# tranqkhue/bugcar_image_segmentation

Hardware: AMD Instinct MI355X
Metric: frames/sec ENet 640x480 segmentation -> BEV occupancy grid (synthetic), whole job (higher is better)
Workload: dtype fp32; 1 GPU; config3/5: ENet 640x480 batch 64 per GPU, preprocess + forward + argmax/LUT + fused BEV warp/occgrid (1000x1000 BEV -> 200x200 cells); global_batch=64, per_gpu_batch=64, height=480, width=640, parallelism=frame-sharded dp1, streams_per_gpu=1, hip_graph=True, ranks=1, devices=1, backend=none (one process)

## Files before the change

__graft_entry__.py:

```python
from __future__ import annotations

import os
import sys

ROOT = os.path.dirname(os.path.abspath(__file__))
if ROOT not in sys.path:
    sys.path.insert(0, ROOT)


def build() -> None:
    from bugcar_image_segmentation_amd.build import build_native
    build_native()
    from oracle.build import build_oracle
    build_oracle()
    import bugcar_image_segmentation_amd
    from bugcar_image_segmentation_amd import _native
    _native.load_library()


def smoke() -> None:
    import numpy as np
    import torch
    from bugcar_image_segmentation_amd import enet_spec, synthetic
    from bugcar_image_segmentation_amd.models import ENET
    from bugcar_image_segmentation_amd.pipeline import OccupancyPipeline
    from oracle import ocv_c

    assert torch.cuda.is_available(), "smoke() needs cuda:0"
    torch.cuda.set_device(0)
    blocks = enet_spec.build_enet()
    H, W = 96, 128
    frames = synthetic.road_frames(2, H, W, seed=3)
    bev = synthetic.synthetic_bev(H, W, 200, 200)
    grid = (4.0, 4.0, 0.05)
    model = ENET(weights=blocks, precision="fp32")
    pipe = OccupancyPipeline(model, bev, *grid, model_hw=(H, W))
    out = pipe.run(torch.from_numpy(frames).cuda()).cpu().numpy()
    x = np.concatenate([ENET.preprocess_device(f, width=W, height=H).cpu().numpy() for f in frames])
    logits = model.logits(x)
    cls_ref, grids_ref, logits_ref = ocv_c.pipeline(frames, blocks, bev._bev_matrix, 200, 200, 1.0, grid, (H, W))
    err = float(np.abs(logits - logits_ref).max())
    assert err < 1e-3, f"logits differ from the oracle by {err}"
    s = np.sort(logits_ref, axis=1)
    thr = max(2.5 * err, 1e-5)
    decided = (s[:, -1] - s[:, -2]) > thr
    cls = model.predict(x)
    assert (cls[decided] == cls_ref[decided]).all(), "class map differs from the oracle"
    seg = pipe._seg.cpu().numpy()
    assert (seg[decided] == cls_ref[decided]).all(), "pipeline class map differs from the oracle"
    own = np.stack([ocv_c.create_occupancy_grid(c, bev._bev_matrix, 200, 200, 1.0, *grid) for c in seg])
    assert (out == own).all(), "occupancy grid differs from the oracle's rasteriser on the same class map"
    from bugcar_image_segmentation_amd import deeplab_spec
    from bugcar_image_segmentation_amd.models import DeepLabV3
    from oracle import deeplab_oracle
    net = deeplab_spec.build_deeplab(width=0.25, crop=65)
    dl = DeepLabV3(net=net, precision="fp32")
    rgb = np.random.default_rng(4).integers(0, 256, (1, 65, 60, 3), dtype=np.uint8)
    seg = dl.predict(rgb)
    dl_logits = dl.logits_device().cpu().numpy()[..., :net.num_classes].transpose(0, 3, 1, 2)
    dl_err = float(np.abs(dl_logits - deeplab_oracle.forward(net, rgb).numpy()).max())
    assert dl_err < 1e-3, f"DeepLab logits differ from the oracle by {dl_err}"
    assert np.array_equal(seg, deeplab_oracle.predict(net, rgb, logits=dl_logits)), "DeepLab resize/argmax differs"
    from bugcar_image_segmentation_amd.models import class_lut3
    net2 = deeplab_spec.build_deeplab(width=0.25, crop=(65, 97))
    dl2 = DeepLabV3(net=net2, precision="fp32")
# ... 91 lines not shown
```

bugcar_image_segmentation_amd/build.py:

```python
from __future__ import annotations

import os
import subprocess
import sys
from concurrent.futures import ThreadPoolExecutor
from pathlib import Path

PKG = Path(__file__).resolve().parent
ROOT = PKG.parent
CSRC = PKG / "csrc"
OBJ = PKG / "_build"
LIB = PKG / "libbugseg.so"
SOURCES = ["conv_kernels.hip", "cls_kernels.hip", "init_kernels.hip", "bneck_kernels.hip", "bneck2_kernels.hip", "up_kernels.hip", "prep_kernels.hip",
           "bev_kernels.hip", "deeplab_kernels.hip", "bugseg_runtime.cpp", "deeplab_runtime.cpp"]
HEADERS = [CSRC / "bugseg_internal.h", CSRC / "deeplab_internal.h", CSRC / "knobs.h", CSRC / "mfma_common.h", CSRC / "cls_common.h", ROOT / "include" / "bugseg.h"]
ARCH = os.environ.get("BUGSEG_OFFLOAD_ARCH", "gfx950")
SOURCE_FLAGS = {"cls_kernels.hip": ["-mllvm", "-amdgpu-mfma-vgpr-form=1"]}


def _hipcc() -> str:
    for c in (os.environ.get("HIPCC"), "/opt/rocm/bin/hipcc", "hipcc"):
        if c and (os.path.sep not in c or os.path.exists(c)):
            return c
    raise RuntimeError("hipcc not found")


def _stale(target: Path, deps) -> bool:
    if not target.exists():
        return True
    t = target.stat().st_mtime
    return any(Path(d).stat().st_mtime > t for d in deps)


def build_native(force: bool = False, verbose: bool = False, stamps: bool = False, variant: str = "",
                 defines=()) -> Path:
    if stamps:
        variant, defines = "stamps", ("-DBUGSEG_STAMPS", *defines)
    obj_dir = OBJ / variant if variant else OBJ
    lib = PKG / f"libbugseg_{variant}.so" if variant else LIB
    obj_dir.mkdir(parents=True, exist_ok=True)
    hipcc = _hipcc()
    flags = [f"--offload-arch={ARCH}", "-O3", "-std=c++17", "-fPIC", "-Wall", "-Wno-unused-function",
             f"-I{ROOT / 'include'}", f"-I{CSRC}", *defines]
    jobs = []
    for s in SOURCES:
        src = CSRC / s
        obj = obj_dir / (s + ".o")
        if force or _stale(obj, [src, *HEADERS]):
            lang = ["-x", "hip"] if s.endswith(".hip") else []
            jobs.append((obj, [hipcc, *flags, *SOURCE_FLAGS.get(s, []), *lang, "-c", str(src), "-o", str(obj)]))

    def run(job):
        obj, cmd = job
        if verbose:
            print(" ".join(cmd), file=sys.stderr)
        r = subprocess.run(cmd, capture_output=True, text=True)
        if r.returncode != 0:
            raise RuntimeError(f"compile failed: {' '.join(cmd)}\n{r.stdout}\n{r.stderr}")
        return obj

    with ThreadPoolExecutor(max_workers=min(4, max(1, len(jobs)))) as ex:
        list(ex.map(run, jobs))
    objs = [obj_dir / (s + ".o") for s in SOURCES]
    if force or jobs or _stale(lib, objs):
        tmp = lib.with_suffix(".so.tmp")
        cmd = [hipcc, f"--offload-arch={ARCH}", "-shared", "-fPIC", "-o", str(tmp), *map(str, objs)]
        r = subprocess.run(cmd, capture_output=True, text=True)
        if r.returncode != 0:
            raise RuntimeError(f"link failed: {' '.join(cmd)}\n{r.stdout}\n{r.stderr}")
        os.replace(tmp, lib)
    return lib


if __name__ == "__main__":
    var = next((a.split("=", 1)[1] for a in sys.argv if a.startswith("--variant=")), "")
    print(build_native(force="--force" in sys.argv, verbose=True, stamps="--stamps" in sys.argv, variant=var,
                       defines=tuple(a for a in sys.argv if a.startswith("-D"))))
```

bugcar_image_segmentation_amd/csrc/bneck_kernels.hip:

```cpp
#include <algorithm>
#include <cstdlib>

#include <type_traits>

#include "bugseg_internal.h"
#ifndef BUGSEG_OUT_AUX
#define BUGSEG_OUT_AUX -1
#endif
#include "cls_common.h"

namespace bugseg {

#ifdef BUGSEG_STAMPS
__device__ unsigned long long *bugseg_stamps;
#define STAMP(k) do { if (tid == 0 && bugseg_stamps) bugseg_stamps[(size_t)tile * 8 + (k)] = __builtin_amdgcn_s_memtime(); } while (0)
#define STAMP_WG() do { if (tid == 0 && bugseg_stamps) bugseg_stamps[(size_t)tile * 8 + 7] = blockIdx.x; } while (0)
#define STAMP_ENTRY(k) do { if (threadIdx.x == 0 && bugseg_stamps) bugseg_stamps[(1u << 19) + 2u * blockIdx.x + (k)] = __builtin_amdgcn_s_memrealtime(); } while (0)
#else
#define STAMP_ENTRY(k) do {} while (0)
#define STAMP(k) do {} while (0)
#define STAMP_WG() do {} while (0)
#endif

__device__ __forceinline__ void vm_wait_upto(int n) {
#define VMW(k) case k: asm volatile("s_waitcnt vmcnt(" #k ")" ::: "memory"); break;
    switch (n) {
        VMW(2) VMW(4) VMW(6) VMW(8) VMW(10) VMW(12) VMW(14) VMW(16) VMW(18) VMW(20) VMW(22) VMW(24)
        default: asm volatile("s_waitcnt vmcnt(0)" ::: "memory"); break;
    }
#undef VMW
}

template <int C, int V> struct BShape;
template <> struct BShape<128, 0> { static constexpr int TH = 16, TW = 16, NW = 8, OCC = 4, RP = 2, RD = 0, WIDE = 1; };
template <> struct BShape<128, 1> { static constexpr int TH = 20, TW = 16, NW = 8, OCC = 4, RP = 2, RD = 0, WIDE = 1; };
template <> struct BShape<128, 2> { static constexpr int TH = 4, TW = 80, NW = 8, OCC = 4, RP = 2, RD = 1, WIDE = 0; };
template <> struct BShape<128, 3> { static constexpr int TH = 4, TW = 64, NW = 8, OCC = 4, RP = 2, RD = 1, WIDE = 1; };
template <> struct BShape<128, 4> { static constexpr int TH = 8, TW = 16, NW = 8, OCC = 4, RP = 1, RD = 0, WIDE = 1; };
template <> struct BShape<64, 0> { static constexpr int TH = 16, TW = 16, NW = 4, OCC = 5, RP = 4, RD = 0, WIDE = 1; };
template <> struct BShape<64, 2> { static constexpr int TH = 8, TW = 16, NW = 4, OCC = 5, RP = 2, RD = 0, WIDE = 1; };
template <> struct BShape<64, 1> { static constexpr int TH = 20, TW = 16, NW = 4, OCC = 5, RP = 3, RD = 0, WIDE = 1; };
template <> struct BShape<16, 0> { static constexpr int TH = 16, TW = 16, NW = 4, OCC = 6, RP = 4, RD = 0, WIDE = 1; };
template <> struct BShape<16, 1> { static constexpr int TH = 20, TW = 16, NW = 4, OCC = 6, RP = 4, RD = 0, WIDE = 1; };

#ifndef BNECK_F32_HL
#define BNECK_F32_HL 1
#endif
#ifndef BNECK_F32_HL64
#define BNECK_F32_HL64 1
#endif
__host__ __device__ constexpr bool bneck_hl(int es, int C, bool dn) {
    return BNECK_F32_HL && es == 4 && (C == 128 || (C == 64 && BNECK_F32_HL64)) && !dn;
}
__host__ __device__ constexpr bool bneck_pl(int es, int C, bool dn) { return bneck_hl(es, C, dn) && C == 64; }
__host__ __device__ constexpr int bneck_padw(int es, int C, bool wide, bool dn) {
    return bneck_hl(es, C, dn) ? 8 : es == 2 && (C != 128 || wide) ? 16 : 16 / es;
}
__host__ __device__ constexpr int bneck_pstr(int es, int IS, bool wide) {
    return es != 2 ? (BNECK_F32_HL && es == 4 && IS == 32 ? 40 : IS + 16 / es) : IS == 32 ? (wide ? 48 : 40) : IS;
}
static bool bneck_wide(int C, int v, bool asym) {
#define BW_CASE(CC, VV) if (C == CC && v == VV) return BShape<CC, VV>::WIDE && !asym;
    BW_CASE(128, 0) BW_CASE(128, 1) BW_CASE(128, 2) BW_CASE(128, 3) BW_CASE(128, 4) BW_CASE(64, 0) BW_CASE(64, 1) BW_CASE(64, 2) BW_CASE(16, 0) BW_CASE(16, 1)
#undef BW_CASE
    return false;
}

int bneck_variants(int C) { return C == 128 ? 6 : C == 16 ? 2 : 3; }

void bneck_shape(int C, int v, int &th, int &tw, int &nw, int *rd) {
    if (C == 128 && v == BNECK2_V) { th = 16; tw = 16; nw = 16; if (rd) *rd = 0; return; }
#define BS_CASE(CC, VV) if (C == CC && v == VV) { th = BShape<CC, VV>::TH; tw = BShape<CC, VV>::TW; nw = BShape<CC, VV>::NW; if (rd) *rd = BShape<CC, VV>::RD; return; }
    BS_CASE(128, 0) BS_CASE(128, 1) BS_CASE(128, 2) BS_CASE(128, 3) BS_CASE(128, 4) BS_CASE(64, 0) BS_CASE(64, 1) BS_CASE(64, 2) BS_CASE(16, 0) BS_CASE(16, 1)
#undef BS_CASE
    th = tw = nw = 0;
    if (rd) *rd = 0;
}

#ifndef BNECK_F32_SPLIT_T0
#define BNECK_F32_SPLIT_T0 1
#endif
#ifndef BNECK_F32_OCC16
#define BNECK_F32_OCC16 4
#endif
// ... 72 lines not shown
#define BNECK_PH2_UNROLL 0
#endif
#ifndef BNECK_ASYM_UNROLL
#define BNECK_ASYM_UNROLL 1
#endif
#ifndef BNECK_REG3_C64
#define BNECK_REG3_C64 0
#endif
#ifndef BNECK_F32_LINES64
#define BNECK_F32_LINES64 0
#endif
#ifndef BNECK_REG3_C64_F32
#define BNECK_REG3_C64_F32 0
#endif
#ifndef BNECK_F32_HSTG
#define BNECK_F32_HSTG 1
#endif
#ifndef BNECK_CH1_C64
#define BNECK_CH1_C64 6
#endif
#ifndef BNECK_CH1_K8
#define BNECK_CH1_K8 1
#endif
#ifndef BNECK_CH1_K8_F32
#define BNECK_CH1_K8_F32 1
#endif
    constexpr int CH1 = KS1 >= 8 ? (sizeof(T) == 4 ? BNECK_CH1_K8_F32 : BNECK_CH1_K8) : KS1 >= 4 ? (NF1 + NW - 1) / NW
                    : KS1 == 2 ? (C == 64 && V == 0 && !DN && !ASYM ? BNECK_CH1_C64 : BNECK_CH1_K2) : 8;
    constexpr bool REG3 = C != 64 || DN || BNECK_REG3_C64 || (sizeof(T) == 4 && (BNECK_REG3_C64_F32 || BNECK_F32_LINES64));
    constexpr bool SWAP = REG3 && sizeof(T) == 2 && NR3 % 2 == 0;
    constexpr bool HALF = REG3 && sizeof(T) == 2 && NR3 % 2 != 0;
    constexpr int EPC = 16 / (int)sizeof(T);
    constexpr int CPP = C / EPC;
    constexpr int CPF = 16 * CPP;
    constexpr int CPL = (CPF + 63) / 64;
    constexpr bool HSTG = !REG3 && sizeof(T) == 4 && C == 64 && BNECK_F32_HSTG;
    constexpr int OSTR = (HSTG ? C / 2 : C) + EPC;
    constexpr int RQ3 = !REG3 ? CPL : SWAP ? NR3 / 2 : NR3;
    static_assert(TW % 16 == 0, "a fragment is a run of one tile row");
#ifndef BNECK_NBE
#define BNECK_NBE -1
#endif
#ifndef BNECK_KEEP
#define BNECK_KEEP 1
#endif
#ifndef BNECK_GLDS
#define BNECK_GLDS 1
#endif
#ifndef BNECK_CONST_GLDS
#define BNECK_CONST_GLDS 1
#endif
#ifndef BNECK_GLDS_PARTIAL
#define BNECK_GLDS_PARTIAL 1
#endif
    constexpr bool GLDS = BNECK_GLDS;
#ifndef BNECK_KEEP_ASYM
#define BNECK_KEEP_ASYM 1
#endif
#ifndef BNECK_KEEP_C64
#define BNECK_KEEP_C64 1
#endif
#ifndef BNECK_KEEP_F32
#define BNECK_KEEP_F32 1
#endif
#ifndef BNECK_KEEP_F32_ASYM
#define BNECK_KEEP_F32_ASYM 1
#endif
    constexpr bool KEEPF = BNECK_KEEP_F32 && !DN && sizeof(T) == 4 && (!ASYM || BNECK_KEEP_F32_ASYM) && C == 128 && REG3 && !SWAP;
    constexpr bool KEEP = (BNECK_KEEP && !DN && sizeof(T) == 2 && (!ASYM || BNECK_KEEP_ASYM) && (SWAP || !REG3) && (C != 64 || BNECK_KEEP_C64) &&
                           NF2 * KS1 * 4 <= (C == 128 ? 48 : 32)) || KEEPF;
    static_assert(!KEEP || !REG3 || (KEEPF ? 2 * KS1 == RQ3 : KS1 == RQ3), "kept x: one 16-B chunk per k-step and row pair");
#ifndef BNECK_EARLY_FREE
#define BNECK_EARLY_FREE 0
#endif
    constexpr bool EARLY_FREE = BNECK_EARLY_FREE && KEEP && REG3;
#ifndef BNECK_DKEEP
#define BNECK_DKEEP 1
#endif
#ifndef BNECK_DKEEP_F32
#define BNECK_DKEEP_F32 1
#endif
    constexpr bool DKEEP = BNECK_DKEEP && DN && ((sizeof(T) == 2 && SWAP) || (sizeof(T) == 4 && BNECK_DKEEP_F32 && REG3));
    constexpr int NPK = DN ? (CI + 31) / 32 : 1;
    constexpr int PKW = sizeof(T) == 4 ? 2 : 1;
#ifndef BNECK_F32_LINES
#define BNECK_F32_LINES 1
#endif
    constexpr bool LINES64 = BNECK_F32_LINES64 && sizeof(T) == 4 && REG3 && C == 64 && !DN && !KEEP;
    constexpr bool LINES = (BNECK_F32_LINES && sizeof(T) == 4 && REG3 && C == 128 && (KEEPF || (DKEEP && PKW == 2)) && RQ3 % 2 == 0) ||
                           LINES64;
    constexpr bool CLS = FC >= 0;
    static_assert(!CLS || (C == 16 && !ASYM && !DN && !TR && REG3 && !KEEP && !SWAP && TH == 16 && TW == 16 && NW == 4),
                  "class fusion: the 16 x 16 C16 form");
    constexpr int OPS = sizeof(T) == 4 ? 20 : 24;
    extern __shared__ __attribute__((aligned(16))) unsigned char smem[];
    using SRaw = typename std::conditional<sizeof(T) == 4 && BNECK_F32_SPLIT_T0, RawS, Raw>::type;
    constexpr bool HL = bneck_hl((int)sizeof(T), C, CI > 0) && !(C == 64 && ASYM);
    static_assert(!HL || (BNECK_F32_SPLIT_T0 && (IS == 32 || (PL && IS == 16)) && BNECK_GLDS), "HL: split t0 of 32 channels (PL: 16), LDS-DMA staging");
    constexpr int PLO = PL ? HR * PSTR : 0;
    constexpr int ZP = HL ? 32 : 16;
    auto st4t = [](T *p, int ch, float4 v) {
        if constexpr (PL) {
            const float e[4] = {v.x, v.y, v.z, v.w};
            _Float16 hh[4], ll[4];
#pragma unroll
            for (int i = 0; i < 4; ++i) {
                hh[i] = (_Float16)e[i];
                ll[i] = (_Float16)(e[i] - (float)hh[i]);
            }
            unsigned char *b = reinterpret_cast<unsigned char *>(reinterpret_cast<float *>(p) - ch) + (ch >> 3) * 16 + (ch & 7) * 2;
            *reinterpret_cast<f16x4 *>(b) = (f16x4){hh[0], hh[1], hh[2], hh[3]};
            *reinterpret_cast<f16x4 *>(b + PLO * 4) = (f16x4){ll[0], ll[1], ll[2], ll[3]};
        } else if constexpr (HL) st4hl(reinterpret_cast<float *>(p) - ch, ch, v);
        else if constexpr (sizeof(T) == 4 && BNECK_F32_SPLIT_T0) st4s(reinterpret_cast<float *>(p) - (ch & 7), ch & 7, v);
        else st4(p, v);
    };

    span_enter(a.span);
    STAMP_ENTRY(0);
    {
        if (tile_walk((int)(blockIdx.x & 7), (int)(blockIdx.x >> 3), tile_walk_ch(a.ntiles), a.ntiles, a.rev) < 0) return true;
    }
    const int tid = threadIdx.x;
    const int lane = tid & 63, col = lane & 15, kq = lane >> 4;
    const int wave = __builtin_amdgcn_readfirstlane(tid >> 6);
    auto chunk_ch = [&](int t) -> int { return SWAP ? (2 * t + (kq & 1)) * 16 + 8 * (kq >> 1) : t * 16 + kq * 4; };
    const int K1S = KS1 * 32 + PADW, K2S = KS2 * 32 + PADW, K3S = 32 + PADW;
    auto ldw = [&](WRaw &r, const T *p) {
        if constexpr (HL) {
            r.h = *reinterpret_cast<const uint4 *>(p + kq * 4);
            r.l = *reinterpret_cast<const uint4 *>(p + 16 + kq * 4);
        } else {
            ld8(r, p + kq * 8);
        }
    };
    T *w1 = reinterpret_cast<T *>(smem);
    T *w2 = w1 + NR1 * 16 * K1S;
    T *w2b = w2 + NR1 * 16 * K2S;
    T *w3 = w2b + (ASYM ? NR1 * 16 * K2S : 0);
    constexpr int NP1 = NR1 * 16;
    float *cb1 = reinterpret_cast<float *>(w3 + C * K3S), *cs1 = cb1 + NP1, *cb2 = cs1 + NP1, *cs2 = cb2 + NP1;
    float *cb2b = cs2 + NP1, *cs2b = cb2b + NP1, *cb3 = cs2b + NP1, *cs3 = cb3 + C, *cso = cs3 + C;
    T *zpad = reinterpret_cast<T *>(cso + C);
    T *ts = zpad + ZP;
    float *wmx = reinterpret_cast<float *>(ts + HR * PSTR);
    T *otile = ts + HR * PSTR;
    uint4 *cwl = reinterpret_cast<uint4 *>(otile + (CLS ? NPX * OPS : 0));
    float *cbl = reinterpret_cast<float *>(cwl + (CLS ? (sizeof(T) == 4 ? 1024 : 512) : 0));
    float *cmx = cbl + 64;
    {
        constexpr int CPR1 = KS1 * 32 * (int)sizeof(T) / 16, CPR2 = KS2 * 32 * (int)sizeof(T) / 16, CPR3 = 32 * (int)sizeof(T) / 16;
        constexpr int N1 = NR1 * 16 * CPR1, N2 = NR1 * 16 * CPR2, N3 = C * CPR3;
        constexpr int TOT = N1 + N2 * (ASYM ? 2 : 1) + N3;
        constexpr int PER = (TOT + NT - 1) / NT;
        uint4 buf[C == 16 ? PER : 1];
        auto locate = [&](int i, const uint4 *&src, unsigned char *&dst) -> bool {
            int r, c;
            if (i < N1) { r = i / CPR1; c = i - r * CPR1; src = (const uint4 *)a.w1 + i; dst = (unsigned char *)(w1 + r * K1S) + c * 16; return true; }
            i -= N1;
            if (i < N2) { r = i / CPR2; c = i - r * CPR2; src = (const uint4 *)a.w2 + i; dst = (unsigned char *)(w2 + r * K2S) + c * 16; return true; }
            i -= N2;
            if (ASYM && i < N2) { r = i / CPR2; c = i - r * CPR2; src = (const uint4 *)a.w2b + i; dst = (unsigned char *)(w2b + r * K2S) + c * 16; return true; }
            if (ASYM) i -= N2;
            if (i < N3) { r = i / CPR3; c = i - r * CPR3; src = (const uint4 *)a.w3 + i; dst = (unsigned char *)(w3 + r * K3S) + c * 16; return true; }
            return false;
        };
        if constexpr (GLDS) {
            (void)buf;
            constexpr int ES = (int)sizeof(T);
            constexpr int SR1 = (KS1 * 32 + PADW) * ES / 16, SR2 = (KS2 * 32 + PADW) * ES / 16, SR3 = (32 + PADW) * ES / 16;
            constexpr int S1 = NR1 * 16 * SR1, S2 = NR1 * 16 * SR2, S3 = C * SR3;
            constexpr int NSL = S1 + S2 * (ASYM ? 2 : 1) + S3;
            static_assert((KS1 * 32 + PADW) * ES % 16 == 0 && (KS2 * 32 + PADW) * ES % 16 == 0 && (32 + PADW) * ES % 16 == 0,
                          "weight rows are whole 16-B slots");
            for (int base = wave * 64; base < NSL; base += NT) {
                const int q = base + lane;
                const uint4 *src;
                auto pick = [&](const void *w, int k, int SR, int CPR) {
                    const int r = k / SR, c = k - r * SR;
                    const int cs = HL ? (c & ~7) | ((c & 7) < 4 ? 2 * (c & 7) : 2 * (c & 3) + 1) : c;
                    src = (const uint4 *)w + r * CPR + (c < CPR ? cs : 0);
                };
                constexpr int O3 = S1 + S2 * (ASYM ? 2 : 1);
                if (q < S1) pick(a.w1, q, SR1, CPR1);
                else if (q < S1 + S2) pick(a.w2, q - S1, SR2, CPR2);
                else if (q < O3) pick(a.w2b, q - S1 - S2, SR2, CPR2);
                else pick(a.w3, q - O3, SR3, CPR3);
                if (base + lane < NSL)
                    __builtin_amdgcn_global_load_lds((__attribute__((address_space(1))) void *)src,
                                                     (__attribute__((address_space(3))) void *)(smem + (size_t)base * 16), 16, 0, 0);
            }
        } else if constexpr (C == 16) {
#pragma unroll
            for (int k = 0; k < PER; ++k) {
                const uint4 *src;
                unsigned char *dst;
                if (locate(tid + k * NT, src, dst)) buf[k] = *src;
            }
#pragma unroll
            for (int k = 0; k < PER; ++k) {
                const uint4 *src;
                unsigned char *dst;
                if (locate(tid + k * NT, src, dst)) *reinterpret_cast<uint4 *>(dst) = buf[k];
            }
        } else {
            (void)buf;
            for (int i = tid; i < TOT; i += NT) {
                const uint4 *src;
                unsigned char *dst;
                if (locate(i, src, dst)) *reinterpret_cast<uint4 *>(dst) = *src;
            }
        }
        if constexpr (GLDS && (BNECK_CONST_GLDS == 2 || (BNECK_CONST_GLDS == 1 && C != 128))) {
            const float *srcs[9] = {a.b1, a.s1, a.b2, a.s2, a.b2b, a.s2b, a.b3, a.s3, a.s_out};
            float *dsts[9] = {cb1, cs1, cb2, cs2, cb2b, cs2b, cb3, cs3, cso};
            int item = 0;
#pragma unroll
            for (int k = 0; k < 9; ++k) {
                if (!ASYM && (k == 4 || k == 5)) continue;
                const int n = k < 6 ? NP1 : C;
#pragma unroll
                for (int c0 = 0; c0 < n; c0 += 64, ++item) {
                    if (item % NW != wave) continue;
                    if (c0 + lane < n)
                        __builtin_amdgcn_global_load_lds((__attribute__((address_space(1))) void *)(srcs[k] + c0 + lane),
                                                         (__attribute__((address_space(3))) void *)(dsts[k] + c0), 4, 0, 0);
                }
            }
        } else {
            for (int i = tid; i < NP1; i += NT) {
                cb1[i] = a.b1[i]; cs1[i] = a.s1[i]; cb2[i] = a.b2[i]; cs2[i] = a.s2[i];
                cb2b[i] = ASYM ? a.b2b[i] : 0.f; cs2b[i] = ASYM ? a.s2b[i] : 0.f;
            }
            for (int i = tid; i < C; i += NT) { cb3[i] = a.b3[i]; cs3[i] = a.s3[i]; cso[i] = a.s_out[i]; }
        }
        if (tid < ZP) zpad[tid] = (T)0.f;
    }
    using CRaw = typename WTr<T>::Raw;
    uint64_t lut64 = 0;
    bool cshort[2] = {false, false};
    if constexpr (CLS) {
        const T *cw = reinterpret_cast<const T *>(a.cw);
        for (int q = tid; q < 512; q += NT) {
            const int bs = q >> 6, ln = q & 63;
            const T *src = cw + (size_t)cls_prow(bs >> 2, ln & 31) * 64 + (bs & 3) * 16 + 8 * (ln >> 5);
            if constexpr (sizeof(T) == 4) {
                cwl[q] = reinterpret_cast<const uint4 *>(src)[0];
                cwl[512 + q] = reinterpret_cast<const uint4 *>(src)[1];
            } else {
                cwl[q] = *reinterpret_cast<const uint4 *>(src);
            }
        }
        if (tid < 64) cbl[tid] = (tid & 15) < a.ncls ? a.cbias[tid] : -INFINITY;
        lut64 = cls_lut64(a.lut);
#pragma unroll
        for (int b = 0; b < 2; ++b) {
            CRaw w2_, w3_;
            const T *r = cw + (size_t)cls_prow(b, lane & 31) * 64 + 8 * (lane >> 5);
            ld8(w2_, r + 32);
            ld8(w3_, r + 48);
            cshort[b] = __ballot(nonzero(w2_) || nonzero(w3_)) == 0;
        }
    }
    const auto rxb = mkbuf(DN ? a.xin : a.x, DN ? a.xin_bytes : a.x_bytes);
    const auto rob = mkbuf(a.out, a.x_bytes);
    const auto rpb = mkbuf(a.pool, a.pool_bytes);
// ... 159 lines not shown
                    __builtin_amdgcn_raw_buffer_store_b64((u32x2_t){lo, hi}, rib, wr ? (int)(pix * a.idxCS + cc * 8) : (int)OOB, 0, 0);
                };
                auto seq = [](float &bv, int &bp, float v, int p) {
                    const bool t = v > bv;
                    bv = t ? v : bv;
                    bp = t ? p : bp;
                };
                if constexpr (CG1 >= 4) {
#pragma unroll
                    for (int hgrp = 0; hgrp < CG1 / 4; ++hgrp) {
                        float bv[8], e[8];
                        int bp[8];
#pragma unroll
                        for (int i = 0; i < 8; ++i) { bv[i] = -INFINITY; bp[i] = 4; }
#pragma unroll
                        for (int tap = 0; tap < 4; ++tap) {
                            elems(xs[tap * (CG1 / 4) + hgrp], e);
#pragma unroll
                            for (int i = 0; i < 8; ++i) seq(bv[i], bp[i], e[i], tap);
                        }
                        emit(hgrp * 4 + kq, bv, bp, interior, hgrp, true);
                    }
                } else {
                    float bv[8], e[8];
                    int bp[8];
#pragma unroll
                    for (int i = 0; i < 8; ++i) { bv[i] = -INFINITY; bp[i] = 4; }
                    const int dx = kq >> 1;
#pragma unroll
                    for (int dy = 0; dy < 2; ++dy) {
                        elems(xs[dy], e);
#pragma unroll
                        for (int i = 0; i < 8; ++i) seq(bv[i], bp[i], e[i], dy * 2 + dx);
                    }
                    const bool lo_half = kq < 2;
#pragma unroll
                    for (int i = 0; i < 8; ++i) {
                        uint32_t v0 = __float_as_uint(bv[i]), v1 = v0, p0 = (uint32_t)bp[i], p1 = p0;
                        pl32swap(v0, v1);
                        pl32swap(p0, p1);
                        const float pv = __uint_as_float(lo_half ? v1 : v0);
                        const int pp = (int)(lo_half ? p1 : p0);
                        const bool t = pv > bv[i] || (pv == bv[i] && pp < bp[i]);
                        bv[i] = t ? pv : bv[i];
                        bp[i] = t ? pp : bp[i];
                    }
                    emit(kq & 1, bv, bp, interior && lo_half, 0, lo_half);
                }
            }
        };
        STAMP(0); STAMP_WG();
        const bool first = it == slot;
        if constexpr (!KEEP) {
            if (GLDS && first) asm volatile("s_waitcnt vmcnt(0)" ::: "memory");
            __syncthreads();
            if constexpr (F32 && !SCL) {
                if (first && bneck_range<ASYM>(a.rg, rng_reduce(rlane)).any) {
                    asm volatile("s_waitcnt vmcnt(0) lgkmcnt(0)" ::: "memory");
                    __syncthreads();
                    return false;
                }
            }
        }
        STAMP(1);

        auto int_h = [&](int f) -> int {
            const int p = f * 16 + col, i = p / TW, j = p - i * TW;
            return (i + RY) * HWW + j + RX;
        };
        auto load_hg = [&](int ty0, int tx0, uint32_t txn, int h, bool valid, Raw (&xs)[KS1]) -> bool {
            const int hy = h / HWW, hx = h - hy * HWW;
            const int iy = ty0 + dt * ((tr ? hx : hy) - RY), ix = tx0 + dtx * ((tr ? hy : hx) - RX);
            const bool ok = valid && (unsigned)iy < (unsigned)a.H && (unsigned)ix < (unsigned)a.W;
#pragma unroll
            for (int s = 0; s < KS1; ++s) {
                const int g = s * 4 + kq;
                bld8(xs[s], rxb, ok && g < G1 ? txn + ((__umul24((uint32_t)iy, (uint32_t)a.W) + (uint32_t)ix) * C + g * 8) * (uint32_t)sizeof(T) : OOB);
            }
            return ok;
        };
        constexpr int NBD = HR - NPX, NFB = (NBD + 15) / 16;
        constexpr int NBW = (NFB + NW - 1) / NW;
        constexpr int B0 = NFT % NW;
        const int wb = wave >= B0 ? wave - B0 : wave - B0 + NW;
        auto bord_h = [&](int b) -> int {
            if (b < 2 * RY * HWW) {
                const int r = b / HWW, c = b - r * HWW;
                return (r < RY ? r : TH + r) * HWW + c;
            }
            if constexpr (RX > 0) {
                const int bb = b - 2 * RY * HWW, r = bb / (2 * RX), c = bb - r * (2 * RX);
                return (RY + r) * HWW + (c < RX ? c : TW + c);
            }
            return 0;
        };
        auto proj = [&](int h, bool valid, bool ok, const Raw (&xs)[KS1]) {
            f32x4 acc[NR1];
            proj_mfma(acc, xs);
            if (valid) {
#pragma unroll
                for (int r = 0; r < NR1; ++r) {
                    const int ch = r * 16 + kq * 4;
                    if (ch >= IS) continue;
                    float4 v = act(f4(acc[r]), cs1 + ch);
                    if (!ok) v = make_float4(0.f, 0.f, 0.f, 0.f);
                    st4t(ts + h * PSTR + ch, ch, v);
                }
            }
        };
        uint4 pres[DKEEP ? NF2 : 1][NPK * PKW];
        if constexpr (KEEP) {
            auto load_h = [&](int h, bool valid, Raw (&xs)[KS1]) -> bool { return load_hg(oy0, ox0, xn, h, valid, xs); };
            Raw bx[NBW][KS1];
            int bh[NBW];
            bool bok[NBW];
            if (!pref) {
#pragma unroll
                for (int j = 0; j < NF2; ++j)
                    if (wave + NW * j < NFT && need1(wave + NW * j)) kok[j] = load_h(int_h(wave + NW * j), true, kx[j]);
            }
            auto load_b = [&](int k) {
                const int b = (wb + NW * k) * 16 + col;
                bh[k] = b < NBD ? bord_h(b) : 0;
                bok[k] = load_h(bh[k], b < NBD, bx[k]);
            };
            constexpr int NBE = BNECK_NBE >= 0 ? BNECK_NBE : C == 128 && !RD && !ASYM && sizeof(T) == 2 ? 1 : 0;
#pragma unroll
            for (int k = 0; k < NBE && k < NBW; ++k)
                if (wb + NW * k < NFB && needb(wb + NW * k)) load_b(k);
            if (GLDS && first) {
                int nld = 0;
                constexpr int LPS = sizeof(T) == 4 ? 2 : 1;
#pragma unroll
                for (int j = 0; j < NF2; ++j) nld += wave + NW * j < NFT && need1(wave + NW * j) ? KS1 * LPS : 0;
#pragma unroll
                for (int k = 0; k < NBE && k < NBW; ++k) nld += wb + NW * k < NFB && needb(wb + NW * k) ? KS1 * LPS : 0;
                vm_wait_upto(BNECK_GLDS_PARTIAL ? (nld < 24 ? nld & ~1 : 24) : 0);
            }
            asm volatile("s_waitcnt lgkmcnt(0)" ::: "memory");
            if (!EARLY_FREE || first) __builtin_amdgcn_s_barrier();
            asm volatile("" ::: "memory");
            if constexpr (F32 && !SCL) {
                if (first && bneck_range<ASYM>(a.rg, rng_reduce(rlane)).any) {
                    asm volatile("s_waitcnt vmcnt(0) lgkmcnt(0)" ::: "memory");
                    __syncthreads();
                    return false;
                }
            }
#pragma unroll
            for (int j = 0; j < NF2; ++j)
                if (wave + NW * j < NFT && need1(wave + NW * j)) proj(int_h(wave + NW * j), true, kok[j], kx[j]);
#pragma unroll
            for (int k = 0; k < NBW; ++k) {
                const int fb = wb + NW * k;
                if (fb >= NFB) break;
                if constexpr (WRD)
                    if (!needb(fb)) continue;
                if (k >= NBE) load_b(k);
                proj(bh[k], fb * 16 + col < NBD, bok[k], bx[k]);
            }
        } else if constexpr (DKEEP) {
            constexpr int NQ = NF2 + NBW;
            auto load_dn = [&](int h, bool valid, Raw (&xs)[KS1]) -> bool {
                const int hy = h / HWW, hx = h - hy * HWW;
                const int iy = oy0 + hy - 1, ix = ox0 + hx - 1;
                const bool ok = valid && (unsigned)iy < (unsigned)a.H && (unsigned)ix < (unsigned)a.W;
#pragma unroll
                for (int s = 0; s < KS1; ++s) {
                    const int g = s * 4 + kq;
                    const int tap = g / CG1, cc = g - tap * CG1;
                    const uint32_t sy = (uint32_t)(2 * iy + (tap >> 1)), sx = (uint32_t)(2 * ix + (tap & 1));
                    uint32_t v = xin_n + ((__umul24(sy, (uint32_t)(2 * a.W)) + sx) * CI + cc * 8) * (uint32_t)sizeof(T);
                    asm volatile("" : "+v"(v));
                    bld8(xs[s], rxb, ok && g < G1 ? v : OOB);
                }
                return ok;
            };
#pragma unroll
            for (int j = 0; j < NF2; ++j)
#pragma unroll
                for (int k = 0; k < NPK * PKW; ++k) pres[j][k] = make_uint4(0u, 0u, 0u, 0u);
#pragma unroll
            for (int q0 = 0; q0 < NQ; q0 += CH1) {
                Raw xf[CH1][KS1];
                bool okc[CH1], vq[CH1];
                int hq[CH1];
#pragma unroll
                for (int c = 0; c < CH1; ++c) {
                    const int q = q0 + c;
                    if (q >= NQ) break;
                    if (q < NF2) {
                        const int f = wave + NW * q;
                        vq[c] = f < NFT;
                        hq[c] = vq[c] ? int_h(f) : 0;
                    } else {
// ... 18 lines not shown
                        proj(hq[c], vq[c], okc[c], xf[c]);
                    }
                }
            }
        } else
        for (int f0 = wave; f0 < NF1; f0 += NW * CH1) {
            Raw xf[CH1][KS1];
            bool okc[CH1];
#pragma unroll
            for (int c = 0; c < CH1; ++c) {
                const int h = (f0 + c * NW) * 16 + col;
                const int hy = h / HWW, hx = h - hy * HWW;
                const int iy = oy0 + dt * ((tr ? hx : hy) - RY), ix = ox0 + dtx * ((tr ? hy : hx) - RX);
                okc[c] = h < HR && (unsigned)iy < (unsigned)a.H && (unsigned)ix < (unsigned)a.W;
#pragma unroll
                for (int s = 0; s < KS1; ++s) {
                    const int g = s * 4 + kq;
                    const bool ld = okc[c] && g < G1;
                    if constexpr (DN) {
                        const int tap = g / CG1, cc = g - tap * CG1;
                        const uint32_t sy = (uint32_t)(2 * iy + (tap >> 1)), sx = (uint32_t)(2 * ix + (tap & 1));
                        uint32_t v = xin_n + ((__umul24(sy, (uint32_t)(2 * a.W)) + sx) * CI + cc * 8) * (uint32_t)sizeof(T);
                        asm volatile("" : "+v"(v));
                        bld8(xf[c][s], rxb, ld ? v : OOB);
                    } else {
                        bld8(xf[c][s], rxb, ld ? xn + ((__umul24((uint32_t)iy, (uint32_t)a.W) + (uint32_t)ix) * C + g * 8) * (uint32_t)sizeof(T) : OOB);
                    }
                }
            }
#pragma unroll
            for (int c = 0; c < CH1; ++c) {
                const int h = (f0 + c * NW) * 16 + col;
                f32x4 acc[NR1];
                proj_mfma(acc, xf[c]);
                if (h < HR) {
#pragma unroll
                    for (int r = 0; r < NR1; ++r) {
                        const int ch = r * 16 + kq * 4;
                        if (ch >= IS) continue;
                        float4 v = act(f4(acc[r]), cs1 + ch);
                        if (!okc[c]) v = make_float4(0.f, 0.f, 0.f, 0.f);
                        st4t(ts + h * PSTR + ch, ch, v);
                    }
                }
                if constexpr (DN) {
                    const int hy = h / HWW, hx = h - hy * HWW;
                    const bool interior = okc[c] && hy >= 1 && hy <= TH && hx >= 1 && hx <= TW;
                    uint4 pkd[NPK * PKW];
                    pool_store(xf[c], interior, oy0 + (hy - 1), ox0 + (hx - 1), pkd);
                }
            }
        }
        STAMP(2);
        __syncthreads();
        STAMP(3);

        constexpr int RP = BShape<C, V>::RP < NF2 ? BShape<C, V>::RP : NF2;
        uint4 res[RP][RQ3];
        auto sc_q = [&](int k) -> int { return HSTG ? lane + 64 * (k % (CPL / 2)) : lane + 64 * k; };
        auto sc_px = [&](int k) -> int { return HSTG ? sc_q(k) / (CPP / 2) : sc_q(k) / CPP; };
        auto sc_ch = [&](int k) -> int {
            return HSTG ? (k / (CPL / 2)) * (CPP / 2) + sc_q(k) % (CPP / 2) : sc_q(k) % CPP;
        };
        auto load_res = [&](int j, uint4 (&r)[RQ3]) {
            if constexpr (!REG3) {
                const int f = wave + NW * j;
#pragma unroll
                for (int k = 0; k < CPL; ++k) {
                    const uint32_t off = res_off(f, sc_px(k), sc_ch(k) * EPC);
                    r[k] = bld16(rrb, HSTG || sc_q(k) < CPF ? off : OOB);
                }
                return;
            }
            if constexpr (LINES64) {
                const uint32_t pc = pix_base(wave + NW * j, col), po8 = pix_base(wave + NW * j, col ^ 8);
                const bool lo8 = col < 8;
                const uint32_t pa = lo8 ? pc : po8, pb = lo8 ? po8 : pc;
#pragma unroll
                for (int u = 0; u < RQ3 / 2; ++u) {
                    const uint32_t cb = (uint32_t)(u * 32 + (lo8 ? 0 : 16) + kq * 4) * (uint32_t)sizeof(T);
                    r[2 * u] = bld16(rrb, pa == OOB ? OOB : pa + cb);
                    r[2 * u + 1] = bld16(rrb, pb == OOB ? OOB : pb + cb);
                }
                return;
            }
            const uint32_t po = DN ? 0u : pix_base(wave + NW * j, col);
#pragma unroll
            for (int t = 0; t < RQ3; ++t) {
                const uint32_t off = DN ? res_off(wave + NW * j, col, chunk_ch(t))
                                        : po == OOB ? OOB : po + (uint32_t)chunk_ch(t) * (uint32_t)sizeof(T);
                if constexpr (HALF) {
                    const u32x2_t v = __builtin_amdgcn_raw_buffer_load_b64(rrb, (int)off, 0, 0);
                    r[t] = make_uint4(v.x, v.y, 0u, 0u);
                } else {
                    r[t] = bld16(rrb, off);
                }
            }
        };
        auto prefetch_res = [&]() {
#pragma unroll
            for (int j = 0; j < RP; ++j) load_res(j, res[j]);
        };
        if constexpr (!ASYM && !KEEP && !DKEEP) prefetch_res();

        Raw tf[NF2];
        auto to_tf = [&](f32x4 (&acc)[NF2][NR1], const float *cs, float om, bool mul) {
// ... 165 lines not shown
                }
                if constexpr (!KEEP) prefetch_res();
                to_tf(acc, cs2b, o2bm, SCL || o2bm != 1.f);
            }
        }

        if constexpr (!REG3) {
            __syncthreads();
            STAMP(5);
            T *stg = ts + wave * 16 * OSTR;
            if constexpr (HSTG) {
                static_assert(!KEEP && CPL % 2 == 0 && NR3 % 2 == 0, "half staging: fp32 C = 64");
#pragma unroll
                for (int j = 0; j < NF2; ++j) {
                    if (wave + NW * j >= NFT) break;
#pragma unroll
                    for (int h = 0; h < 2; ++h) {
#pragma unroll
                        for (int kk = 0; kk < CPL / 2; ++kk) {
                            const int k = h * (CPL / 2) + kk;
                            *reinterpret_cast<uint4 *>(stg + sc_px(k) * OSTR + (sc_ch(k) - h * (CPP / 2)) * EPC) = res[j % RP][k];
                        }
                        if (h == 1 && j + RP < NF2 && wave + NW * (j + RP) < NFT) load_res(j + RP, res[j % RP]);
                        wave_lds_sync();
#pragma unroll
                        for (int rr = 0; rr < NR3 / 2; ++rr) {
                            const int r = h * (NR3 / 2) + rr;
                            const int ch = r * 16 + kq * 4;
                            static_assert(bias_in_acc(NR3, 1), "expansion: one k step, bias in the accumulator");
                            f32x4 acc = bias_m(cb3 + ch, b3m, SCL || scl);
                            WRaw wf;
                            ldw(wf, w3 + (r * 16 + col) * K3S);
                            mma(acc, wf, tf[j]);
                            T *sp = stg + col * OSTR + (ch - h * (C / 2));
                            float4 v = f4(acc);
                            if constexpr (F32) {
                                if (scl) v = mul4(v, o3m);
                            }
                            v = act(v, cs3 + ch);
                            v = act(add4(v, ld4(sp)), cso + ch);
                            if constexpr (F32) rng_acc4(amo, v);
                            st4(sp, v);
                        }
                        wave_lds_sync();
#pragma unroll
                        for (int kk = 0; kk < CPL / 2; ++kk) {
                            const int k = h * (CPL / 2) + kk;
                            const uint32_t off = pix_off(wave + NW * j, sc_px(k), sc_ch(k) * EPC);
                            bst16o<OAUX>(rob, off, *reinterpret_cast<const uint4 *>(stg + sc_px(k) * OSTR + (sc_ch(k) - h * (CPP / 2)) * EPC));
                        }
                        wave_lds_sync();
                    }
                }
                STAMP(6);
                continue;
            }
#pragma unroll
            for (int j = 0; j < NF2; ++j) {
                if (wave + NW * j >= NFT) break;
                if constexpr (KEEP) {
#pragma unroll
                    for (int s = 0; s < KS1; ++s)
                        if (s * 4 + kq < G1) *reinterpret_cast<uint4 *>(stg + col * OSTR + (s * 4 + kq) * EPC) = kx[j][s].v;
                } else {
#pragma unroll
                    for (int k = 0; k < CPL; ++k) {
                        const int q = lane + 64 * k;
                        if (q < CPF) *reinterpret_cast<uint4 *>(stg + (q / CPP) * OSTR + (q % CPP) * EPC) = res[j % RP][k];
                    }
                    if (j + RP < NF2 && wave + NW * (j + RP) < NFT) load_res(j + RP, res[j % RP]);
                }
                wave_lds_sync();
#pragma unroll
                for (int r = 0; r < NR3; ++r) {
                    const int ch = r * 16 + kq * 4;
                    f32x4 acc = bias_m(cb3 + ch, b3m, SCL || scl);
                    WRaw wf;
                    ldw(wf, w3 + (r * 16 + col) * K3S);
                    mma(acc, wf, tf[j]);
                    T *sp = stg + col * OSTR + ch;
                    float4 v = f4(acc);
                    if constexpr (F32) {
                        if (scl) v = mul4(v, o3m);
                    }
                    v = act(v, cs3 + ch);
                    v = act(add4(v, ld4(sp)), cso + ch);
                    if constexpr (F32) rng_acc4(amo, v);
                    st4(sp, v);
                }
                wave_lds_sync();
#pragma unroll
                for (int k = 0; k < CPL; ++k) {
                    const int q = lane + 64 * k;
                    if (q < CPF) {
                        const uint32_t off = pix_off(wave + NW * j, q / CPP, (q % CPP) * EPC);
                        bst16o<OAUX>(rob, off, *reinterpret_cast<const uint4 *>(stg + (q / CPP) * OSTR + (q % CPP) * EPC));
                    }
                }
                wave_lds_sync();
            }
            STAMP(6);
            continue;
        }
        if constexpr (EARLY_FREE) __syncthreads();
        STAMP(5);
#pragma unroll
        for (int j = 0; j < NF2; ++j) {
            if (wave + NW * j >= NFT) break;
            if constexpr (WRD)
                if (!live(wave + NW * j)) continue;
            const uint32_t po = pix_base(wave + NW * j, col);
            auto to_quads = [&](RawF &k) {
                uint32_t a[4] = {__float_as_uint(k.a.x), __float_as_uint(k.a.y), __float_as_uint(k.a.z), __float_as_uint(k.a.w)};
                uint32_t b[4] = {__float_as_uint(k.b.x), __float_as_uint(k.b.y), __float_as_uint(k.b.z), __float_as_uint(k.b.w)};
#pragma unroll
                for (int d = 0; d < 4; ++d) {
                    pl16swap(a[d], b[d]);
                    pl32swap(a[d], b[d]);
                }
                k.a = make_float4(__uint_as_float(a[0]), __uint_as_float(a[1]), __uint_as_float(a[2]), __uint_as_float(a[3]));
                k.b = make_float4(__uint_as_float(b[0]), __uint_as_float(b[1]), __uint_as_float(b[2]), __uint_as_float(b[3]));
            };
            if constexpr (DKEEP && PKW == 2) {
#pragma unroll
                for (int s = 0; s < NPK; ++s) to_quads(reinterpret_cast<RawF &>(pres[j][2 * s]));
            }
            if constexpr (KEEPF) {
#pragma unroll
                for (int s = 0; s < KS1; ++s) to_quads(reinterpret_cast<RawF &>(kx[j][s]));
            }
            auto out3 = [&](int r, const f32x4 &acc) {
                const int ch = r * 16 + kq * 4;
                float4 v = f4(acc);
                if constexpr (F32) {
                    if (scl) v = mul4(v, o3m);
                }
                return act(v, cs3 + ch);
            };
            if constexpr (LINES) {
                const uint32_t po_o = pix_base(wave + NW * j, col ^ 8);
                const bool lo8 = col < 8;
                const uint32_t pa = lo8 ? po : po_o, pb = lo8 ? po_o : po;
#pragma unroll
                for (int u = 0; u < RQ3 / 2; ++u) {
                    float4 v2[2];
                    uint4 rl[2];
                    if constexpr (LINES64) {
                        const uint4 l1 = res[j % RP][2 * u], l2 = res[j % RP][2 * u + 1];
                        const uint4 xs = lo8 ? l2 : l1;
                        uint4 ys;
                        ys.x = (uint32_t)__builtin_amdgcn_update_dpp(0, (int)xs.x, 0x128, 0xf, 0xf, false);
                        ys.y = (uint32_t)__builtin_amdgcn_update_dpp(0, (int)xs.y, 0x128, 0xf, 0xf, false);
                        ys.z = (uint32_t)__builtin_amdgcn_update_dpp(0, (int)xs.z, 0x128, 0xf, 0xf, false);
// ... 140 lines not shown
                    int off = ((i + dy) * TW + jj + dx) * OPS + 8 * hh;
                    asm volatile("" : "+v"(off));
                    ld8(xq, ok ? otile + off : zpad);
                };
                int cls[2];
#pragma unroll
                for (int b = 0; b < 2; ++b) {
                    f32x16 acc;
                    const float4 *bb = reinterpret_cast<const float4 *>(cbl + (2 * b + hh) * 16);
#pragma unroll
                    for (int q = 0; q < 4; ++q) {
                        const float4 v = bb[q];
                        acc[4 * q] = v.x; acc[4 * q + 1] = v.y; acc[4 * q + 2] = v.z; acc[4 * q + 3] = v.w;
                    }
                    auto taps = [&](auto sc) {
#pragma unroll
                        for (int s = 0; s < 4; ++s) {
                            if (s >= 2 && cshort[b]) break;
                            CRaw w;
                            if constexpr (sizeof(T) == 4) {
                                w.h = cwl[(b * 4 + s) * 64 + ln];
                                w.l = cwl[512 + (b * 4 + s) * 64 + ln];
                            } else {
                                w.v = cwl[(b * 4 + s) * 64 + ln];
                            }
                            Raw xq;
                            tap_x(s, xq);
                            if constexpr (decltype(sc)::value) mul8(reinterpret_cast<RawF &>(xq), xm);
                            mma32(acc, w, xq);
                        }
                    };
                    bool done = false;
                    if constexpr (F32) {
                        if (csc) {
#pragma unroll
                            for (int c = 0; c < 16; ++c) acc[c] *= bm;
                            taps(std::true_type());
#pragma unroll
                            for (int c = 0; c < 16; ++c) acc[c] *= om;
                            done = true;
                        }
                    }
                    if (!done) taps(std::false_type());
                    cls[b] = cls_argmax1<(FC < 0 ? 0 : FC)>(acc, lut64);
                }
                uint32_t c0 = (uint32_t)cls[0], c1 = (uint32_t)cls[1];
                pl32swap(c0, c1);
                const bool valid = i < TH - 1 && jj < TW - 1 && y < a.H && x < a.W;
                const uint32_t o = (uint32_t)n * plane + (uint32_t)(2 * y + hh) * W2 + 2u * (uint32_t)x;
                __builtin_amdgcn_raw_buffer_store_b16((unsigned short)(c0 | (c1 << 8)), rcls, valid ? (int)o : (int)OOB, 0, 0);
            }
        }
        pref = has_next;
        STAMP(6);
    }
    if constexpr (F32) rng_commit_wg(amo, a.rg.amax_out, reinterpret_cast<float *>(ts), NW);
    span_exit(a.span);
    STAMP_ENTRY(1);
    return true;
}

template <typename T, int C, bool ASYM, int V, bool TR, int CI = 0>
__global__ void __launch_bounds__((BShape<C, V>::NW * 64), (sizeof(T) == 2 ? BShape<C, V>::OCC : C == 16 ? BNECK_F32_OCC16 : C == 64 ? (V == 2 ? BNECK_F32_OCC64_V2 : BNECK_F32_OCC64) : BNECK_F32_OCC128)) bneck_kernel(const BneckArgs a) {
    if constexpr (sizeof(T) == 4) {
        const float rl = rng_lane(a.rg);
        if (!bneck_body<T, C, ASYM, V, TR, CI, false>(a, rl)) bneck_body<T, C, ASYM, V, TR, CI, true>(a, rl);
    } else {
        bneck_body<T, C, ASYM, V, TR, CI, false>(a, 0.f);
    }
}

template <typename T, int C, bool ASYM, int V>
__global__ void __launch_bounds__((BShape<C, V>::NW * 64), BNECK_F32_OCC128) bneck_win_kernel(const BneckArgs a) {
    static_assert(sizeof(T) == 4 && C == 128, "windowed forms: fp32 C = 128");
    const float rl = rng_lane(a.rg);
    if (!bneck_body<T, C, ASYM, V, false, 0, false, -1, true>(a, rl)) bneck_body<T, C, ASYM, V, false, 0, true, -1, true>(a, rl);
}

template <typename T, int FC>
__global__ void __launch_bounds__(256, (sizeof(T) == 2 ? BShape<16, 0>::OCC : BNECK_F32_OCC16)) bneck_cls_kernel(const BneckArgs a) {
    if constexpr (sizeof(T) == 4) {
        const float rl = rng_lane(a.rg);
        if (!bneck_body<T, 16, false, 0, false, 0, false, FC>(a, rl)) bneck_body<T, 16, false, 0, false, 0, true, FC>(a, rl);
    } else {
        bneck_body<T, 16, false, 0, false, 0, false, FC>(a, 0.f);
    }
}

#ifdef BUGSEG_STAMPS
extern "C" int bugseg_debug_set_stamps(void *p) {
    return hipMemcpyToSymbol(HIP_SYMBOL(bugseg_stamps), &p, sizeof(p)) == hipSuccess ? 0 : -3;
}
#endif

bool bneck_keeps_c64(int prec, int v) { return BNECK_KEEP_C64 && prec != PREC_F32 && v != 1; }

size_t bneck_lds_bytes(int prec, int C, bool asym, int v, int cin, bool cls) {
    if (C == 128 && v == BNECK2_V) return prec == PREC_F32 && !asym && cin == 0 ? bneck2_lds_bytes() : (size_t)1 << 30;
    int TH, TW, NW, RD;
    bneck_shape(C, v, TH, TW, NW, &RD);
    const int es = prec_es(prec), pad = 16 / es;
    const int I = cin > 0 ? cin / 4 : C / 4, IS = I < 8 ? 8 : I, NR1 = (I + 15) / 16;
    const int KS1 = ((cin > 0 ? cin / 2 : C / 8) + 3) / 4, KS2 = ((asym ? 5 : 9) * IS / 8 + 3) / 4;
    const int R = asym ? 2 : 1, RX = RD ? 0 : R;
    const bool wide = bneck_wide(C, v, asym);
    const int padw = bneck_padw(es, C, wide, cin > 0);
// ... 112 lines not shown
```

Before: 22680 frames/s.

## Order bottleneck weight staging so stage-1 weights land first with partial waits

New measurement: 22800 frames/s (median of 6 runs). Within noise of the previous version (+0.6%).

```diff
diff --git a/__graft_entry__.py b/__graft_entry__.py
--- a/__graft_entry__.py
+++ b/__graft_entry__.py
@@ -9,8 +9,9 @@
 
 
 def build() -> None:
-    from bugcar_image_segmentation_amd.build import build_native
+    from bugcar_image_segmentation_amd.build import build_native, order0_lib
     build_native()
+    order0_lib()
     from oracle.build import build_oracle
     build_oracle()
     import bugcar_image_segmentation_amd
diff --git a/bugcar_image_segmentation_amd/build.py b/bugcar_image_segmentation_amd/build.py
--- a/bugcar_image_segmentation_amd/build.py
+++ b/bugcar_image_segmentation_amd/build.py
@@ -33,10 +33,13 @@
 
 
 def build_native(force: bool = False, verbose: bool = False, stamps: bool = False, variant: str = "",
-                 defines=()) -> Path:
+                 defines=(), only=()) -> Path:
     if stamps:
         variant, defines = "stamps", ("-DBUGSEG_STAMPS", *defines)
     obj_dir = OBJ / variant if variant else OBJ
+    only = tuple(only) if variant else ()
+    if only:
+        build_native(verbose=verbose)
     lib = PKG / f"libbugseg_{variant}.so" if variant else LIB
     obj_dir.mkdir(parents=True, exist_ok=True)
     hipcc = _hipcc()
@@ -44,6 +47,8 @@
              f"-I{ROOT / 'include'}", f"-I{CSRC}", *defines]
     jobs = []
     for s in SOURCES:
+        if only and s not in only:
+            continue
         src = CSRC / s
         obj = obj_dir / (s + ".o")
         if force or _stale(obj, [src, *HEADERS]):
@@ -61,7 +66,7 @@
 
     with ThreadPoolExecutor(max_workers=min(4, max(1, len(jobs)))) as ex:
         list(ex.map(run, jobs))
-    objs = [obj_dir / (s + ".o") for s in SOURCES]
+    objs = [(obj_dir if not only or s in only else OBJ) / (s + ".o") for s in SOURCES]
     if force or jobs or _stale(lib, objs):
         tmp = lib.with_suffix(".so.tmp")
         cmd = [hipcc, f"--offload-arch={ARCH}", "-shared", "-fPIC", "-o", str(tmp), *map(str, objs)]
@@ -72,7 +77,15 @@
     return lib
 
 
+def order0_lib() -> Path:
+    lib = PKG / "libbugseg_order0.so"
+    if _stale(lib, [*(CSRC / s for s in SOURCES), *HEADERS]):
+        lib = build_native(variant="order0", defines=("-DBNECK_STAGE_ORDER=0",), only=("bneck_kernels.hip",))
+    return lib
+
+
 if __name__ == "__main__":
     var = next((a.split("=", 1)[1] for a in sys.argv if a.startswith("--variant=")), "")
     print(build_native(force="--force" in sys.argv, verbose=True, stamps="--stamps" in sys.argv, variant=var,
-                       defines=tuple(a for a in sys.argv if a.startswith("-D"))))
+                       defines=tuple(a for a in sys.argv if a.startswith("-D")),
+                       only=tuple(a.split("=", 1)[1] for a in sys.argv if a.startswith("--only="))))
diff --git a/bugcar_image_segmentation_amd/csrc/bneck_kernels.hip b/bugcar_image_segmentation_amd/csrc/bneck_kernels.hip
--- a/bugcar_image_segmentation_amd/csrc/bneck_kernels.hip
+++ b/bugcar_image_segmentation_amd/csrc/bneck_kernels.hip
@@ -30,6 +30,30 @@
     }
 #undef VMW
 }
+__device__ __forceinline__ void vm_wait_upto62(int n) {
+#define VMW(k) case k: asm volatile("s_waitcnt vmcnt(" #k ")" ::: "memory"); break;
+    switch (n > 62 ? 62 : n & ~1) {
+        VMW(2) VMW(4) VMW(6) VMW(8) VMW(10) VMW(12) VMW(14) VMW(16) VMW(18) VMW(20) VMW(22) VMW(24) VMW(26) VMW(28) VMW(30) VMW(32)
+        VMW(34) VMW(36) VMW(38) VMW(40) VMW(42) VMW(44) VMW(46) VMW(48) VMW(50) VMW(52) VMW(54) VMW(56) VMW(58) VMW(60) VMW(62)
+        default: asm volatile("s_waitcnt vmcnt(0)" ::: "memory"); break;
+    }
+#undef VMW
+}
+template <int ENC>
+__device__ __forceinline__ void vm_wait_seen() {
+    asm volatile("" ::: "memory");
+    __builtin_amdgcn_s_waitcnt(ENC);
+    asm volatile("" ::: "memory");
+}
+#pragma clang diagnostic push
+#pragma clang diagnostic ignored "-Winline-asm"
+__device__ __forceinline__ void glds_asm16(const void *src, uint32_t lds) {
+    asm volatile("s_mov_b32 m0, %1\n\ts_nop 0\n\tglobal_load_lds_dwordx4 %0, off" : : "v"(src), "s"(lds) : "memory", "m0");
+}
+__device__ __forceinline__ void glds_asm4(const void *src, uint32_t lds) {
+    asm volatile("s_mov_b32 m0, %1\n\ts_nop 0\n\tglobal_load_lds_dword %0, off" : : "v"(src), "s"(lds) : "memory", "m0");
+}
+#pragma clang diagnostic pop
 
 template <int C, int V> struct BShape;
 template <> struct BShape<128, 0> { static constexpr int TH = 16, TW = 16, NW = 8, OCC = 4, RP = 2, RD = 0, WIDE = 1; };
@@ -208,6 +232,12 @@
 #endif
 #ifndef BNECK_GLDS_PARTIAL
 #define BNECK_GLDS_PARTIAL 1
+#endif
+#ifndef BNECK_ORD_LATCH
+#define BNECK_ORD_LATCH 1
+#endif
+#ifndef BNECK_STAGE_ORDER
+#define BNECK_STAGE_ORDER 1
 #endif
     constexpr bool GLDS = BNECK_GLDS;
 #ifndef BNECK_KEEP_ASYM
@@ -304,6 +334,33 @@
     uint4 *cwl = reinterpret_cast<uint4 *>(otile + (CLS ? NPX * OPS : 0));
     float *cbl = reinterpret_cast<float *>(cwl + (CLS ? (sizeof(T) == 4 ? 1024 : 512) : 0));
     float *cmx = cbl + 64;
+    constexpr bool ORD = BNECK_STAGE_ORDER && BNECK_GLDS && sizeof(T) == 4 && !CLS && (BNECK_STAGE_ORDER == 2 || KEEP);
+    constexpr bool ORDC = ORD && BNECK_CONST_GLDS != 0;
+    constexpr int OSR1 = (KS1 * 32 + PADW) * (int)sizeof(T) / 16, OSR2 = (KS2 * 32 + PADW) * (int)sizeof(T) / 16;
+    constexpr int ONSL = NR1 * 16 * OSR1 + NR1 * 16 * OSR2 * (ASYM ? 2 : 1) + C * (32 + PADW) * (int)sizeof(T) / 16;
+    constexpr int OSB = (NR1 * 16 * OSR1 + 63) & ~63;
+    static_assert(!ORD || OSB <= ONSL, "part A lies inside the weight region");
+    auto ord_consts = [&](bool late, auto &&f) -> int {
+        int item = 0, cnt = 0;
+#pragma unroll
+        for (int k = 0; k < 9; ++k) {
+            if (!ASYM && (k == 4 || k == 5)) continue;
+            const int n = k < 6 ? NP1 : C;
+#pragma unroll
+            for (int c0 = 0; c0 < n; c0 += 64, ++item) {
+                if ((k >= 2) != late || item % NW != wave) continue;
+                ++cnt;
+                f(k, c0, n);
+            }
+        }
+        return cnt;
+    };
+    auto ord_late = [&]() -> int {
+        const int nw = OSB + wave * 64 < ONSL ? (ONSL - OSB - wave * 64 + NT - 1) / NT : 0;
+        return nw + (ORDC ? ord_consts(true, [](int, int, int) {}) : 0);
+    };
+    if constexpr (ORD && !SCL)
+        if (bneck_range<ASYM>(a.rg, rng_reduce(rlane)).any) return false;
     {
         constexpr int CPR1 = KS1 * 32 * (int)sizeof(T) / 16, CPR2 = KS2 * 32 * (int)sizeof(T) / 16, CPR3 = 32 * (int)sizeof(T) / 16;
         constexpr int N1 = NR1 * 16 * CPR1, N2 = NR1 * 16 * CPR2, N3 = C * CPR3;
@@ -321,7 +378,37 @@
             if (i < N3) { r = i / CPR3; c = i - r * CPR3; src = (const uint4 *)a.w3 + i; dst = (unsigned char *)(w3 + r * K3S) + c * 16; return true; }
             return false;
         };
-        if constexpr (GLDS) {
+        if constexpr (ORD) {
+            (void)buf;
+            vm_wait_seen<0x0F70>();
+            constexpr int O2 = NR1 * 16 * OSR1, O2B = O2 + NR1 * 16 * OSR2, O3 = O2 + NR1 * 16 * OSR2 * (ASYM ? 2 : 1);
+            auto slots = [&](int lo, int hi) {
+                for (int base = lo + wave * 64; base < hi; base += NT) {
+                    const int q = base + lane;
+                    const uint4 *src;
+                    auto pick = [&](const void *w, int k, int SR, int CPR) {
+                        const int r = k / SR, c = k - r * SR;
+                        const int cs = HL ? (c & ~7) | ((c & 7) < 4 ? 2 * (c & 7) : 2 * (c & 3) + 1) : c;
+                        src = (const uint4 *)w + r * CPR + (c < CPR ? cs : 0);
+                    };
+                    if (q < O2) pick(a.w1, q, OSR1, CPR1);
+                    else if (q < O2B) pick(a.w2, q - O2, OSR2, CPR2);
+                    else if (q < O3) pick(a.w2b, q - O2B, OSR2, CPR2);
+                    else pick(a.w3, q - O3, (32 + PADW) * (int)sizeof(T) / 16, CPR3);
+                    if (q < ONSL)
+                        glds_asm16(src, (uint32_t)(size_t)(__attribute__((address_space(3))) void *)(smem + (size_t)base * 16));
+                }
+            };
+            const float *srcs[9] = {a.b1, a.s1, a.b2, a.s2, a.b2b, a.s2b, a.b3, a.s3, a.s_out};
+            float *dsts[9] = {cb1, cs1, cb2, cs2, cb2b, cs2b, cb3, cs3, cso};
+            auto cdma = [&](int k, int c0, int n) {
+                if (c0 + lane < n) glds_asm4(srcs[k] + c0 + lane, (uint32_t)(size_t)(__attribute__((address_space(3))) void *)(dsts[k] + c0));
+            };
+            slots(0, OSB);
+            if constexpr (ORDC) ord_consts(false, cdma);
+            slots(OSB, ONSL);
+            if constexpr (ORDC) ord_consts(true, cdma);
+        } else if constexpr (GLDS) {
             (void)buf;
             constexpr int ES = (int)sizeof(T);
             constexpr int SR1 = (KS1 * 32 + PADW) * ES / 16, SR2 = (KS2 * 32 + PADW) * ES / 16, SR3 = (32 + PADW) * ES / 16;
@@ -367,7 +454,8 @@
                 if (locate(i, src, dst)) *reinterpret_cast<uint4 *>(dst) = *src;
             }
         }
-        if constexpr (GLDS && (BNECK_CONST_GLDS == 2 || (BNECK_CONST_GLDS == 1 && C != 128))) {
+        if constexpr (ORDC) {
+        } else if constexpr (GLDS && (BNECK_CONST_GLDS == 2 || (BNECK_CONST_GLDS == 1 && C != 128))) {
             const float *srcs[9] = {a.b1, a.s1, a.b2, a.s2, a.b2b, a.s2b, a.b3, a.s3, a.s_out};
             float *dsts[9] = {cb1, cs1, cb2, cs2, cb2b, cs2b, cb3, cs3, cso};
             int item = 0;
@@ -633,9 +721,12 @@
         STAMP(0); STAMP_WG();
         const bool first = it == slot;
         if constexpr (!KEEP) {
-            if (GLDS && first) asm volatile("s_waitcnt vmcnt(0)" ::: "memory");
+            if (GLDS && first) {
+                if constexpr (ORD) vm_wait_upto62(ord_late());
+                else asm volatile("s_waitcnt vmcnt(0)" ::: "memory");
+            }
             __syncthreads();
-            if constexpr (F32 && !SCL) {
+            if constexpr (F32 && !SCL && !ORD) {
                 if (first && bneck_range<ASYM>(a.rg, rng_reduce(rlane)).any) {
                     asm volatile("s_waitcnt vmcnt(0) lgkmcnt(0)" ::: "memory");
                     __syncthreads();
@@ -716,12 +807,13 @@
                 for (int j = 0; j < NF2; ++j) nld += wave + NW * j < NFT && need1(wave + NW * j) ? KS1 * LPS : 0;
 #pragma unroll
                 for (int k = 0; k < NBE && k < NBW; ++k) nld += wb + NW * k < NFB && needb(wb + NW * k) ? KS1 * LPS : 0;
-                vm_wait_upto(BNECK_GLDS_PARTIAL ? (nld < 24 ? nld & ~1 : 24) : 0);
+                if constexpr (ORD) vm_wait_upto62(BNECK_GLDS_PARTIAL ? nld + ord_late() : 0);
+                else vm_wait_upto(BNECK_GLDS_PARTIAL ? (nld < 24 ? nld & ~1 : 24) : 0);
             }
             asm volatile("s_waitcnt lgkmcnt(0)" ::: "memory");
             if (!EARLY_FREE || first) __builtin_amdgcn_s_barrier();
             asm volatile("" ::: "memory");
-            if constexpr (F32 && !SCL) {
+            if constexpr (F32 && !SCL && !ORD) {
                 if (first && bneck_range<ASYM>(a.rg, rng_reduce(rlane)).any) {
                     asm volatile("s_waitcnt vmcnt(0) lgkmcnt(0)" ::: "memory");
                     __syncthreads();
@@ -846,6 +938,7 @@
             }
         }
         STAMP(2);
+        if constexpr (ORD) { if (first) asm volatile("s_waitcnt vmcnt(0)" ::: "memory"); }
         __syncthreads();
         STAMP(3);
 
@@ -1117,6 +1210,7 @@
                         wave_lds_sync();
                     }
                 }
+                if constexpr (ORD && BNECK_ORD_LATCH) vm_wait_seen<0x0F70>();
                 STAMP(6);
                 continue;
             }
@@ -1164,6 +1258,7 @@
                 }
                 wave_lds_sync();
             }
+            if constexpr (ORD && BNECK_ORD_LATCH) vm_wait_seen<0x0F70>();
             STAMP(6);
             continue;
         }
@@ -1410,6 +1505,7 @@
             }
         }
         pref = has_next;
+        if constexpr (ORD && BNECK_ORD_LATCH) vm_wait_seen<0x0F70>();
         STAMP(6);
     }
     if constexpr (F32) rng_commit_wg(amo, a.rg.amax_out, reinterpret_cast<float *>(ts), NW);
```
